# LazyLatte/vortex-raytracing

Measured on AMD Instinct MI355X. Metric: Mrays/s (primary+shadow) at 1920x1080, 1M-tri BVH, higher is better.
Workload: dtype f32; 1 GPU; configs[2]: Sponza-class 1048576 tris, 1920x1080, primary + 1 shadow ray per hit; frames_in_flight=2, frames_per_launch_group=5, parallelism=1 GPU: whole frames, 5 per set of launches (vxrt_render_batch), 2 sets in flight, world_size=1, bvh_nodes=726810, bvh_depth=13

## Files before the change

### vortex-raytracing_amd/build.py

```python
import os
import shutil
import struct
import subprocess
import sys

HERE = os.path.dirname(os.path.abspath(__file__))
CSRC = os.path.join(HERE, "csrc")
LIB = os.path.join(HERE, "lib")
VXBIN = os.path.join(HERE, "vxbin")
ROCM = os.environ.get("ROCM_PATH", "/opt/rocm")
HIPCC = os.path.join(ROCM, "bin", "hipcc")
ARCH = "gfx950"

HIP_FLAGS = ["--offload-arch=" + ARCH, "-O3", "-ffp-contract=off", "-fno-slp-vectorize", "-fPIC", "-std=c++17", "-Wall", "-Wno-unused-function"]
HIP_FLAGS += os.environ.get("VXRT_EXTRA_HIPFLAGS", "").split()
CXX_FLAGS = ["-O2", "-ffp-contract=off", "-fPIC", "-std=c++17", "-Wall"]

PRODUCT_HIP_SOURCES = ("rt_kernels.hip", "rt_accel.hip", "rt_secondary.hip", "rt_path.hip", "rt_denoise.hip", "rc_kernels.hip", "vx_backend.hip", "bvh_builder.hip")


def hip_library_deps():
    incs = sorted(f for f in os.listdir(CSRC) if f.endswith((".h", ".inc")))
    return [os.path.join(CSRC, f) for f in PRODUCT_HIP_SOURCES + tuple(incs)] + [os.path.join(HERE, "..", "include", "vortex_hip.h")]

SELECTORS = {
    "kernel": (0x80000000, "raytracing.kernel"),
    "miss": (0x80100000, "raytracing.miss"),
    "closest": (0x80200000, "raytracing.closest"),
    "anyhit": (0x80300000, "raytracing.anyhit"),
    "raycast/kernel": (0x80000000, "raycast.kernel"),
}


def _newer(target, sources):
    if not os.path.exists(target):
        return True
    t = os.path.getmtime(target)
    return any(os.path.getmtime(s) > t for s in sources)


def _run(cmd):
    print("+", " ".join(cmd), flush=True)
    subprocess.check_call(cmd)


def write_selectors():
    os.makedirs(VXBIN, exist_ok=True)
    for name, (vma, tag) in SELECTORS.items():
        payload = ("VXHIP1:" + tag).encode() + b"\0"
        payload += b"\0" * (64 - len(payload))
        blob = struct.pack("<QQ", vma, vma + 0x1000) + payload
        os.makedirs(os.path.dirname(os.path.join(VXBIN, name)), exist_ok=True)
        with open(os.path.join(VXBIN, name + ".vxbin"), "wb") as f:
            f.write(blob)


TEST_VARIANT_FLAGS = ["-DRT_TOP_NODES=84", "-DRT_LDS_STACK_RENDER=5", "-DRT_LDS_STACK_RENDER_PACKED=4", "-DRT_TRI_LDS=4", "-DRT_TRI_LDS_MIN=2", "-DRT_ORDER_CHECK=1"]


def build_test_variant(force=False):
    d = os.path.join(HERE, "lib_ab", "lds_staging")
    os.makedirs(d, exist_ok=True)
    so = os.path.join(d, "libvortex-hip.so")
    src = [os.path.join(CSRC, f) for f in PRODUCT_HIP_SOURCES]
    if force or _newer(so, hip_library_deps()):
        _run([HIPCC] + HIP_FLAGS + TEST_VARIANT_FLAGS + ["-shared", "-o", so] + src)
    for f in ("libvortex.so", "libvxrt_scene.so"):
        shutil.copy2(os.path.join(LIB, f), os.path.join(d, f))
    return d


def build(force=False, verbose=True):
    os.makedirs(LIB, exist_ok=True)
    hdrs = hip_library_deps()
    if not os.path.exists(HIPCC):
        raise RuntimeError("hipcc not found at %s: the HIP path cannot be built" % HIPCC)

    hip_so = os.path.join(LIB, "libvortex-hip.so")
    hip_src = [os.path.join(CSRC, f) for f in PRODUCT_HIP_SOURCES]
    if force or _newer(hip_so, hdrs):
        _run([HIPCC] + HIP_FLAGS + ["-shared", "-o", hip_so] + hip_src)

    cal_so = os.path.join(LIB, "libvxrt_calib.so")
    cal_src = [os.path.join(CSRC, "calib_kernels.hip")]
    if force or _newer(cal_so, cal_src):
        _run([HIPCC] + HIP_FLAGS + ["-shared", "-o", cal_so] + cal_src)

    stub_so = os.path.join(LIB, "libvortex.so")
    stub_src = [os.path.join(CSRC, "vx_stub.cpp")]
    if force or _newer(stub_so, stub_src + hdrs):
        _run(["g++"] + CXX_FLAGS + ["-shared", "-o", stub_so] + stub_src + ["-ldl"])

    scene_so = os.path.join(LIB, "libvxrt_scene.so")
    scene_src = [os.path.join(CSRC, "scene_builder.cpp")]
    if force or _newer(scene_so, scene_src + hdrs):
        _run(["g++"] + CXX_FLAGS + ["-pthread", "-shared", "-o", scene_so] + scene_src + ["-lz"])

    host = os.path.join(LIB, "rt_host")
    host_src = [os.path.join(CSRC, "rt_host.cpp")]
    if os.path.exists(host_src[0]) and (force or _newer(host, host_src + hdrs + [stub_so, scene_so])):
        _run(["g++"] + CXX_FLAGS + ["-o", host] + host_src + ["-L" + LIB, "-lvortex", "-lvxrt_scene", "-pthread", "-Wl,-rpath,$ORIGIN"])

    write_selectors()
    build_test_variant(force)
    return {"hip": hip_so, "stub": stub_so, "scene": scene_so}


if __name__ == "__main__":
    build(force="--force" in sys.argv)
```

### vortex-raytracing_amd/csrc/rt_kernels.hip

```cpp
#include <hip/hip_runtime.h>
#include <stdint.h>
#include "rt_internal.h"
#include "pinhole.h"
#include "rt_shading.h"
#include "rt_order.h"

template <bool EXACT>
__device__ __forceinline__ float slab_interval(float tx1, float tx2, float ty1, float ty2, float tz1, float tz2) {
  float tmin, tmax;
  if (EXACT) {
    tmin = std_min(tx1, tx2);
    tmax = std_max(tx1, tx2);
    tmin = std_max(tmin, std_min(ty1, ty2));
    tmax = std_min(tmax, std_max(ty1, ty2));
    tmin = std_max(tmin, std_min(tz1, tz2));
    tmax = std_min(tmax, std_max(tz1, tz2));
  } else {
    tmin = fmaxf(fmaxf(fminf(tx1, tx2), fminf(ty1, ty2)), fminf(tz1, tz2));
    tmax = fminf(fminf(fmaxf(tx1, tx2), fmaxf(ty1, ty2)), fmaxf(tz1, tz2));
  }
  return (tmax < tmin || tmax <= 0) ? RT_LARGE_FLOAT : tmin;
}

template <bool EXACT>
// ... 117 lines not shown
  }
  const uint32_t desc[4] = {q2.z, q2.w, q3.x, q3.y};
  float d[4];
  bool in[4] = {true, true, true, true};
  if constexpr (NO_SELECT) {
    static_assert(!EXACT && !LDEXP, "the select-free box test is the fast form's");
    d[0] = child_box_raw<0>(pl, px, py, pz, sx, sy, sz, rox, roy, roz, rix, riy, riz, in[0]);
    d[1] = child_box_raw<1>(pl, px, py, pz, sx, sy, sz, rox, roy, roz, rix, riy, riz, in[1]);
    d[2] = child_box_raw<2>(pl, px, py, pz, sx, sy, sz, rox, roy, roz, rix, riy, riz, in[2]);
    d[3] = child_box_raw<3>(pl, px, py, pz, sx, sy, sz, rox, roy, roz, rix, riy, riz, in[3]);
  } else {
    d[0] = child_box<0, EXACT, LDEXP>(pl, px, py, pz, sx, sy, sz, ex, ey, ez, rox, roy, roz, rix, riy, riz);
    d[1] = child_box<1, EXACT, LDEXP>(pl, px, py, pz, sx, sy, sz, ex, ey, ez, rox, roy, roz, rix, riy, riz);
    d[2] = child_box<2, EXACT, LDEXP>(pl, px, py, pz, sx, sy, sz, ex, ey, ez, rox, roy, roz, rix, riy, riz);
    d[3] = child_box<3, EXACT, LDEXP>(pl, px, py, pz, sx, sy, sz, ex, ey, ez, rox, roy, roz, rix, riy, riz);
  }
#pragma unroll
  for (int k = 0; k < 4; ++k) {
    if constexpr (NO_SELECT) ok[k] = (desc[k] != DESC_NONE) && in[k] && (d[k] < hit_dist);
    else ok[k] = (desc[k] != DESC_NONE) && (d[k] < hit_dist);
    c[k].d = d[k];
    c[k].desc = desc[k];
  }
}

template <bool EXACT, bool LDEXP>
__device__ __forceinline__ void eval_children(const uint4 q0, const uint4 q1, const uint4 q2, const uint4 q3, const uint32_t* __restrict__ ref_node,
                                              float rox, float roy, float roz, float rix, float riy, float riz,
                                              float hit_dist, Cand* c) {
  bool ok[4];
  eval_children_raw<EXACT, LDEXP>(q0, q1, q2, q3, ref_node, rox, roy, roz, rix, riy, riz, hit_dist, c, ok);
#pragma unroll
  for (int k = 0; k < 4; ++k) c[k].d = ok[k] ? c[k].d : __builtin_inff();
}

struct Fetches { unsigned node = 0, inst = 0, tri = 0; };

#define ITER_LIMIT (1u << 22)

template <int N>
__device__ __forceinline__ float* cam_lds() { __shared__ float s[N]; return s; }

#ifndef RT_TRI_PREFETCH
#define RT_TRI_PREFETCH 1
#endif
#ifndef RT_WAVES_PER_EU
#define RT_WAVES_PER_EU 6
#endif

#ifndef RT_DEAD_MAX
#define RT_DEAD_MAX 64
#endif
#ifndef RT_LEAF_MIN
#define RT_LEAF_MIN 1
#endif
#ifndef RT_TRACE_LEAF_MIN
#define RT_TRACE_LEAF_MIN 24
#endif
#ifndef RT_TRI_LDS
#define RT_TRI_LDS 0
#endif
#ifndef RT_TRI_LDS_MIN
#define RT_TRI_LDS_MIN 8
#endif
#ifndef RT_UNORDERED_OCCLUSION
#define RT_UNORDERED_OCCLUSION 1
#endif
#ifndef RT_SHADOW_FINISH_MIN
#define RT_SHADOW_FINISH_MIN 65
#endif
#ifndef RT_TRACE_DEAD_MAX
#define RT_TRACE_DEAD_MAX 16
#endif
#ifndef RT_CHUNK
#define RT_CHUNK 64
#endif
#ifndef RT_TRACE_NT
#define RT_TRACE_NT 0
#endif
#ifndef RT_TRACE_CHUNK
#define RT_TRACE_CHUNK 64
#endif
#ifndef RT_XCC_HOME
#define RT_XCC_HOME 1
#endif
#ifndef RT_QUEUE_DRY_MASK
#define RT_QUEUE_DRY_MASK 1
#endif
#ifndef RT_STEAL_SPREAD
#define RT_STEAL_SPREAD 0
#endif
#ifndef RT_WAVES_TRACE
#define RT_WAVES_TRACE 7
#endif
#ifndef RT_LDS_STACK_TRACE
#define RT_LDS_STACK_TRACE 7
#endif
#ifndef RT_WAVES_RENDER
#define RT_WAVES_RENDER 7
#endif
#ifndef RT_LDS_STACK_RENDER
#define RT_LDS_STACK_RENDER 6
#endif
#ifndef RT_WAVES_RENDER_PACKED
#define RT_WAVES_RENDER_PACKED 8
#endif
#ifndef RT_LDS_STACK_RENDER_PACKED
#define RT_LDS_STACK_RENDER_PACKED 5
#endif
#ifndef LDS_STACK
#define LDS_STACK 8
#endif
#ifndef RT_WG_WAVES
#define RT_WG_WAVES 4
#endif
#define RT_WG_THREADS (64 * RT_WG_WAVES)

enum { JOB_RENDER = 0, JOB_RENDER_SHADOW = 1, JOB_TRACE = 2, JOB_RENDER_GI = 3, JOB_TRACE_UNORDERED = 4 };
__host__ __device__ constexpr bool is_trace_job(int job) { return job == JOB_TRACE || job == JOB_TRACE_UNORDERED; }
enum { JOB_CAM = 8 };
__host__ __device__ constexpr int job_base(int job) { return job & ~JOB_CAM; }
__host__ __device__ constexpr bool is_cam_job(int job) { return (job & JOB_CAM) != 0; }
#ifndef RT_WAVES_GI
#define RT_WAVES_GI 7
#endif
#ifndef RT_LDS_STACK_GI
#define RT_LDS_STACK_GI 6
#endif
#ifndef RT_GI_DEAD_MAX
#define RT_GI_DEAD_MAX 64
#endif

#ifndef RT_BATCH_PUSH
#define RT_BATCH_PUSH 1
#endif
#ifndef RT_LEAF_FLAT
#define RT_LEAF_FLAT 1
#endif
#ifndef RT_OCC_OK_MASKS
#define RT_OCC_OK_MASKS 1
#endif
#ifndef RT_OCC_LOOP
#define RT_OCC_LOOP 1
#endif
#ifndef RT_OCC_LOOP_CHECK
#define RT_OCC_LOOP_CHECK 0
#endif
#ifndef RT_ORDER_PATHS
#define RT_ORDER_PATHS 1
#endif
#ifndef RT_ORDER_CHECK
#define RT_ORDER_CHECK 0
#endif

#ifdef RT_ISA_MARKS
#define RT_MARK(name) asm volatile("; RTMARK " name)
#else
#define RT_MARK(name)
#endif
#define RT_LOOP_MARK(name) do { if constexpr (OCC) { RT_MARK("occ_" name); } else { RT_MARK(name); } } while (0)

__device__ __forceinline__ uint32_t frame_row(uint32_t lr, uint32_t y0, uint32_t row_step) { return y0 + (lr >> 3) * row_step + (lr & 7u); }

struct FastDiv { uint32_t d, m, s; };
static FastDiv fast_div_make(uint32_t d) {
  FastDiv f{d ? d : 1u, 1u, 0u};
  while ((1ull << f.s) < f.d) ++f.s;
  f.m = (uint32_t)((((1ull << f.s) - f.d) << 32) / f.d) + 1u;
  return f;
}
__device__ __forceinline__ uint32_t fast_div(uint32_t x, const FastDiv& f) { return (__umulhi(x, f.m) + x) >> f.s; }

struct PersistArgs {
  uint32_t W, H, y0, y1, tiles_x;
  FastDiv div_tiles_x, div_frame_tiles;
  uint32_t row_step;
  uint32_t total;
  const uint32_t* total_dev;
  HitRec* hits;
  const float* rays; const float* tmax; int any_hit;
  const uint32_t* order;
  unsigned long long* counters;
  uint32_t* status;
  uint32_t* queue;
  uint32_t per_shard;
  const float* utab; const float* vtab;
  uint32_t* defer_count; uint32_t* defer_list; uint32_t defer_cap;
  const uint32_t* tile_order; uint32_t* tile_cost;
  uint32_t shard_rot;
  unsigned long long* wave_log;
  unsigned long long* end_log;
  const ShadeParams* pbatch; uint32_t frame_tiles;
  uint32_t* dst; float* colors; uint32_t gi_seed;
  const uint8_t* alpha_tri;
};

#define RT_FAST_INV_MAX 0x1p+64f
#define RT_FAST_POS_MAX 0x1p+60f
__device__ __forceinline__ bool ray_in_fast_domain(float ox, float oy, float oz, float ix, float iy, float iz) {
  return fabsf(ix) <= RT_FAST_INV_MAX && fabsf(iy) <= RT_FAST_INV_MAX && fabsf(iz) <= RT_FAST_INV_MAX && ix != 0.0f && iy != 0.0f && iz != 0.0f &&
         fabsf(ox) <= RT_FAST_POS_MAX && fabsf(oy) <= RT_FAST_POS_MAX && fabsf(oz) <= RT_FAST_POS_MAX;
}


#define F_FOUND 1u
#define F_ANYHIT 2u
#define F_SHADOW 8u
#define F_WORLD 16u
#define F_RESUMED 32u

__device__ unsigned long long g_child_counts[8];

template <int JOB, int STATS, bool LDEXP, bool EXACT, bool PACKED = false, bool SHALLOW = false, bool ALPHA = false, bool IDENT = false>
__global__ __launch_bounds__(EXACT ? 256 : RT_WG_THREADS, EXACT ? 4 : (is_trace_job(JOB) ? RT_WAVES_TRACE : (job_base(JOB) == JOB_RENDER_GI ? RT_WAVES_GI : (PACKED ? RT_WAVES_RENDER_PACKED : RT_WAVES_RENDER)))) void rt_persistent_kernel(SceneDev sc, ShadeParams p, PersistArgs A) {
  static_assert(!ALPHA || (STATS == 0 && !PACKED && !SHALLOW && job_base(JOB) != JOB_RENDER_GI), "alpha instantiations: see ALPHA above");
  static_assert(!IDENT || (STATS == 0 && !ALPHA && !EXACT && !LDEXP && SHALLOW && (job_base(JOB) == JOB_RENDER || job_base(JOB) == JOB_RENDER_SHADOW)), "identity-root instantiations: see IDENT above");
  constexpr int LSTK = EXACT ? LDS_STACK : (is_trace_job(JOB) ? RT_LDS_STACK_TRACE : (job_base(JOB) == JOB_RENDER_GI ? RT_LDS_STACK_GI : (PACKED ? RT_LDS_STACK_RENDER_PACKED : RT_LDS_STACK_RENDER)));
  constexpr int WG_WAVES = EXACT ? 4 : RT_WG_WAVES;
  constexpr bool USE_TOP = RT_TOP_NODES > 0 && !EXACT && !LDEXP;
  constexpr uint32_t DEAD_MAX = is_trace_job(JOB) ? RT_TRACE_DEAD_MAX : (job_base(JOB) == JOB_RENDER_GI ? RT_GI_DEAD_MAX : RT_DEAD_MAX);
  constexpr uint32_t FINISH_MIN = job_base(JOB) == JOB_RENDER_SHADOW ? RT_SHADOW_FINISH_MIN : 65u;
  const uint32_t lane = threadIdx.x & 63u;
  const uint32_t n_jobs = EXACT ? min(*A.defer_count, A.defer_cap) : (A.total_dev ? min(*A.total_dev, A.total) : A.total);
  const uint32_t per_shard = (EXACT || A.total_dev) ? (((n_jobs + QUEUE_SHARDS - 1) / QUEUE_SHARDS + 63u) & ~63u) : A.per_shard;

  __shared__ uint2 s_stk[WG_WAVES][LSTK][64];
  constexpr int NCTX = (!EXACT && is_trace_job(JOB)) ? 8 : 9;
  __shared__ uint32_t s_ctx[WG_WAVES][NCTX][64];
  __shared__ uint32_t s_dry;
  if (threadIdx.x == 0) s_dry = 0u;
  float* s_cam = nullptr;
  if constexpr (is_cam_job(JOB)) {
    s_cam = cam_lds<CAM_TAB>();
    for (uint32_t i = threadIdx.x; i < (uint32_t)CAM_TAB; i += blockDim.x) s_cam[i] = A.utab[i];
  }
  __syncthreads();
  uint2* const lstk = &s_stk[threadIdx.x >> 6][0][lane];
  auto lstk4_here = [&]() -> uint32_t* {
    uint32_t l = lane;
    asm volatile("" : "+v"(l));
    return (uint32_t*)lstk - l;
  };
  uint32_t* const ctx = &s_ctx[threadIdx.x >> 6][0][lane];
#define CTX(i) ctx[((NCTX == 8 && (i) > 5) ? (i) - 1 : (i)) * 64]
  __shared__ uint4 s_top[USE_TOP ? 4 : 1][USE_TOP ? RT_TOP_NODES : 1];
  constexpr bool TRI_LDS = RT_TRI_LDS > 0 && !EXACT && !is_trace_job(JOB);
  __shared__ float4 s_tri[TRI_LDS ? WG_WAVES : 1][TRI_LDS ? 3 * RT_TRI_LDS : 1];
  const uint32_t n_top = USE_TOP ? min(sc.n_top, (uint32_t)RT_TOP_NODES) : 0u;
  if (USE_TOP && n_top) {
    for (uint32_t i = threadIdx.x; i < 4u * n_top; i += (uint32_t)(64 * WG_WAVES)) s_top[i / n_top][i % n_top] = sc.top_img[(size_t)(i / n_top) * RT_TOP_NODES + (i % n_top)];
    __syncthreads();
  }
  const uint32_t root_desc = (USE_TOP && n_top) ? sc.tlas_root_top : sc.tlas_root;
  const uint32_t* const blas_roots = (USE_TOP && n_top) ? sc.blas_root_top : sc.blas_root;
  const uint32_t root_blas_desc = is_inst_desc(root_desc) ? blas_roots[root_desc & PAYLOAD_MASK] : DESC_DONE;

  float arx = 0, ary = 0, arz = 0, aix = 0, aiy = 0, aiz = 0;
  float hitd = 0, path_m = 0, tos_m = 0;
  uint32_t cur = DESC_IDLE, tos_d = DESC_DONE, job = 0, flags = 0;
  float g_col[3] = {0.f, 0.f, 0.f}, g_alb[3] = {0.f, 0.f, 0.f}, g_ray[6] = {0.f, 0.f, 0.f, 0.f, 0.f, 0.f};
  int sp = 0;
  constexpr int STACK_CAP = SHALLOW ? 3 * RT_SHALLOW_LEVELS : LSTK + RT_STACK_ENTRIES;
  static_assert(STACK_CAP > LSTK, "stack");
  uint32_t ovf_d[STACK_CAP - LSTK];
  float ovf_m[STACK_CAP - LSTK];
  constexpr bool BOX_NO_SELECT = RT_BOX_NO_SELECT && RT_OCC_OK_MASKS && IDENT && job_base(JOB) == JOB_RENDER_SHADOW;
  constexpr bool OCC_LOOP = RT_OCC_LOOP && IDENT && RT_BATCH_PUSH && RT_UNORDERED_OCCLUSION && RT_OCC_OK_MASKS && job_base(JOB) == JOB_RENDER_SHADOW &&
                            DEAD_MAX >= 64u && FINISH_MIN > 64u && STACK_CAP > 2 * LSTK;
  bool queue_empty = false;
  const uint32_t xcc_id = RT_XCC_HOME ? (uint32_t)__builtin_amdgcn_s_getreg((3 << 11) | (0 << 6) | 20) : blockIdx.x;
  const uint32_t shard = (xcc_id + A.shard_rot) % QUEUE_SHARDS;
  uint32_t tries = 0, loc_next = 0, loc_end = 0;
  uint32_t loc_off = 0;
  uint32_t lpt_tile = 0xFFFFFFFFu, lpt_work = 0; unsigned long long lpt_t0 = 0;
  Fetches fx;
  unsigned nrays = 0, nhit = 0;
  unsigned long long t_first = 0;
  unsigned long long wl_tn = 0, wl_tl = 0, wl_t0 = 0;
  unsigned wl_no23 = 0, wl_no3 = 0, wl_iter = 0, wl_node_x = 0, wl_node_l = 0, wl_leaf_x = 0, wl_leaf_l = 0;
  unsigned wl_cc[8] = {0, 0, 0, 0, 0, 0, 0, 0};
  unsigned long long wl_tstart = 0, wl_tf = 0, wl_tfin = 0, wl_tmark = 0;
  unsigned long long wl_tq = 0;
  if (STATS && A.wave_log) { t_first = wall_clock64(); wl_tstart = __builtin_readcyclecounter(); }

  auto pixel_of = [&](uint32_t r, uint32_t& x, uint32_t& y) {
    asm volatile("" : "+v"(r));
    uint32_t tile = r >> 6;
    const uint32_t l = r & 63u;
    if (A.pbatch) tile -= fast_div(tile, A.div_frame_tiles) * A.frame_tiles;
    const uint32_t ty = fast_div(tile, A.div_tiles_x);
    x = (tile - ty * A.tiles_x) * 8u + (l & 7u);
    y = A.y0 + ty * A.row_step + (l >> 3);
  };
  auto hit_slot = [&]() -> HitRec* {
    uint32_t j = job;
    asm volatile("" : "+v"(j));
    return A.hits + j;
  };
  auto pixel_ray = [&](uint32_t x, uint32_t y, float& ox, float& oy, float& oz, float& dx, float& dy, float& dz) {
    if constexpr (is_cam_job(JOB)) {
      const uint32_t f = A.pbatch ? fast_div(job >> 6, A.div_frame_tiles) : 0u;
      camera_ray(s_cam + f * CAM_HDR, A.vtab + (size_t)f * (A.W + A.H), A.W, x, y, ox, oy, oz, dx, dy, dz);
    } else generate_ray(A.utab[x], A.vtab[y], ox, oy, oz, dx, dy, dz);
  };
  auto world_ray = [&](float& ox, float& oy, float& oz, float& dx, float& dy, float& dz, float& tmax_) {
    tmax_ = RT_LARGE_FLOAT;
    if (is_trace_job(JOB)) {
      const float* rp = A.rays + (size_t)job * 6;
      if (RT_TRACE_NT) {
        ox = __builtin_nontemporal_load(rp); oy = __builtin_nontemporal_load(rp + 1); oz = __builtin_nontemporal_load(rp + 2);
        dx = __builtin_nontemporal_load(rp + 3); dy = __builtin_nontemporal_load(rp + 4); dz = __builtin_nontemporal_load(rp + 5);
      } else { ox = rp[0]; oy = rp[1]; oz = rp[2]; dx = rp[3]; dy = rp[4]; dz = rp[5]; }
      if (A.tmax) tmax_ = A.tmax[job];
    } else {
      uint32_t x, y;
      pixel_of(job, x, y);
      pixel_ray(x, y, ox, oy, oz, dx, dy, dz);
      if (job_base(JOB) == JOB_RENDER_GI && (flags & F_SHADOW)) {
        ox = g_ray[0]; oy = g_ray[1]; oz = g_ray[2]; dx = g_ray[3]; dy = g_ray[4]; dz = g_ray[5];
      }
      if (job_base(JOB) == JOB_RENDER_SHADOW && (flags & F_SHADOW)) {
        const float pd = __uint_as_float(CTX(5));
        float sox, soy, soz, sdx, sdy, sdz, sdist;
        float lpx = p.lpos[0], lpy = p.lpos[1], lpz = p.lpos[2];
        if (A.pbatch) { const ShadeParams* q = A.pbatch + fast_div(job >> 6, A.div_frame_tiles); lpx = q->lpos[0]; lpy = q->lpos[1]; lpz = q->lpos[2]; }
        shadow_ray(lpx, lpy, lpz, ox, oy, oz, dx, dy, dz, pd, sox, soy, soz, sdx, sdy, sdz, sdist);
        ox = sox; oy = soy; oz = soz; dx = sdx; dy = sdy; dz = sdz;
        tmax_ = sdist;
      }
    }
  };
  auto defer = [&](bool counted) {
    const uint32_t slot = atomicAdd(A.defer_count, 1u);
    if (job_base(JOB) == JOB_RENDER_GI && (flags & F_SHADOW)) nrays--;
    if (slot < A.defer_cap) A.defer_list[slot] = job | ((flags & F_SHADOW) && job_base(JOB) != JOB_RENDER_GI ? 0x80000000u : 0u);
    if (job_base(JOB) == JOB_RENDER_SHADOW && (flags & F_SHADOW)) {
      HitRec h;
      h.bx = __uint_as_float(CTX(3)); h.by = __uint_as_float(CTX(4)); h.bz = 1 - h.bx - h.by;
      h.dist = __uint_as_float(CTX(5)); h.blasIdx = CTX(6); h.triIdx = CTX(7);
      *hit_slot() = h;
    }
    if (counted) nrays--;
    cur = DESC_IDLE;
  };
  auto enter_instance = [&](uint32_t blasIdx, float ox, float oy, float oz, float dx, float dy, float dz) {
    const uint32_t* bp = sc.blas + (size_t)blasIdx * (RT_BLAS_STRIDE / 4);
    uint32_t bw[13];
#pragma unroll
    for (int i = 0; i < 13; ++i) bw[i] = bp[i];
    if (STATS) { fx.node++; fx.inst++; }
    const float m00 = __uint_as_float(bw[1]), m01 = __uint_as_float(bw[2]), m02 = __uint_as_float(bw[3]), m03 = __uint_as_float(bw[4]);
    const float m10 = __uint_as_float(bw[5]), m11 = __uint_as_float(bw[6]), m12 = __uint_as_float(bw[7]), m13 = __uint_as_float(bw[8]);
    const float m20 = __uint_as_float(bw[9]), m21 = __uint_as_float(bw[10]), m22 = __uint_as_float(bw[11]), m23 = __uint_as_float(bw[12]);
    arx = m00 * ox + m01 * oy + m02 * oz + m03;
    ary = m10 * ox + m11 * oy + m12 * oz + m13;
    arz = m20 * ox + m21 * oy + m22 * oz + m23;
    const float cdx = m00 * dx + m01 * dy + m02 * dz;
    const float cdy = m10 * dx + m11 * dy + m12 * dz;
    const float cdz = m20 * dx + m21 * dy + m22 * dz;
    aix = 1.0f / cdx; aiy = 1.0f / cdy; aiz = 1.0f / cdz;
    const bool s2 = ray_in_fast_domain(arx, ary, arz, aix, aiy, aiz);
    if (!EXACT && !s2) { defer(true); return; }
    flags &= ~F_WORLD;
    CTX(0) = __float_as_uint(cdx); CTX(1) = __float_as_uint(cdy); CTX(2) = __float_as_uint(cdz);
    CTX(8) = blasIdx;
    cur = blas_roots[blasIdx];
  };
  auto start_ray = [&](float ox, float oy, float oz, float dx, float dy, float dz, float tmax_, bool any_) {
    arx = ox; ary = oy; arz = oz;
    aix = 1.0f / dx; aiy = 1.0f / dy; aiz = 1.0f / dz;
    const bool safe = ray_in_fast_domain(ox, oy, oz, aix, aiy, aiz);
    flags = (flags & (F_SHADOW | F_RESUMED)) | F_WORLD | (any_ ? F_ANYHIT : 0u);
    if (!EXACT && !safe) {
      if (!is_trace_job(JOB) && !is_cam_job(JOB) && !(flags & F_SHADOW)) cur = DESC_IDLE; else defer(false);
      return;
    }
    hitd = tmax_ > RT_LARGE_FLOAT ? RT_LARGE_FLOAT : tmax_;
    path_m = -__builtin_inff(); sp = 0; tos_d = DESC_DONE;
    cur = root_desc;
    nrays++;
    if (is_inst_desc(root_desc)) {
      const bool no_neg_zero = __float_as_uint(ox) != 0x80000000u && __float_as_uint(oy) != 0x80000000u && __float_as_uint(oz) != 0x80000000u;
      if (sc.ident_root && safe && no_neg_zero) {
        if (STATS) { fx.node++; fx.inst++; }
        flags &= ~F_WORLD;
        CTX(0) = __float_as_uint(dx); CTX(1) = __float_as_uint(dy); CTX(2) = __float_as_uint(dz);
        CTX(8) = root_desc & PAYLOAD_MASK;
        cur = root_blas_desc;
      } else enter_instance(root_desc & PAYLOAD_MASK, ox, oy, oz, dx, dy, dz);
    }
  };
  volatile uint32_t* const vovf_d = ovf_d;
  volatile float* const vovf_m = ovf_m;
  auto push = [&](uint32_t d, float m) {
    if (tos_d != DESC_DONE) {
      if (sp < LSTK) lstk[sp * 64] = make_uint2(tos_d, __float_as_uint(tos_m));
      else { ovf_d[sp - LSTK] = tos_d; ovf_m[sp - LSTK] = tos_m; }
      ++sp;
    }
    tos_d = d; tos_m = m;
  };
  auto push_pending = [&](auto occ, bool p0, uint32_t d0, float m0, bool p1, uint32_t d1, float m1, bool p2, uint32_t d2, float m2) {
    constexpr bool OCC = decltype(occ)::value;
    if (!RT_BATCH_PUSH) {
      if (p0) push(d0, m0);
      if (p1) push(d1, m1);
      if (p2) push(d2, m2);
      return;
    }
    if (!(p0 || p1 || p2)) return;
    const bool w_top = tos_d != DESC_DONE;
    const bool w0 = p0 && (p1 || p2), w1 = p1 && p2;
    const int q0 = sp + (w_top ? 1 : 0), q1 = q0 + (w0 ? 1 : 0), end = q1 + (w1 ? 1 : 0);
    if constexpr (OCC) {
      constexpr int LROWS = 2 * LSTK;
      uint32_t* const lstk4 = lstk4_here();
      if (end <= LROWS) {
        if (w_top) lstk4[sp * 64] = tos_d;
        if (w0) lstk4[q0 * 64] = d0;
        if (w1) lstk4[q1 * 64] = d1;
      } else if (sp >= LROWS) {
        if (w_top) ovf_d[sp - LROWS] = tos_d;
        if (w0) ovf_d[q0 - LROWS] = d0;
        if (w1) ovf_d[q1 - LROWS] = d1;
      } else {
        auto put = [&](int q, uint32_t d) {
          if (q < LROWS) lstk4[q * 64] = d;
          else ovf_d[q - LROWS] = d;
        };
        if (w_top) put(sp, tos_d);
        if (w0) put(q0, d0);
        if (w1) put(q1, d1);
      }
    } else
    if (end <= LSTK) {
      if (w_top) lstk[sp * 64] = make_uint2(tos_d, __float_as_uint(tos_m));
      if (w0) lstk[q0 * 64] = make_uint2(d0, __float_as_uint(m0));
      if (w1) lstk[q1 * 64] = make_uint2(d1, __float_as_uint(m1));
    } else if (sp >= LSTK) {
      if (w_top) { ovf_d[sp - LSTK] = tos_d; ovf_m[sp - LSTK] = tos_m; }
      if (w0) { ovf_d[q0 - LSTK] = d0; ovf_m[q0 - LSTK] = m0; }
      if (w1) { ovf_d[q1 - LSTK] = d1; ovf_m[q1 - LSTK] = m1; }
    } else {
      auto put = [&](int q, uint32_t d, float m) {
        if (q < LSTK) lstk[q * 64] = make_uint2(d, __float_as_uint(m));
        else { ovf_d[q - LSTK] = d; ovf_m[q - LSTK] = m; }
      };
      if (w_top) put(sp, tos_d, tos_m);
      if (w0) put(q0, d0, m0);
      if (w1) put(q1, d1, m1);
    }
    sp = end;
    tos_d = p2 ? d2 : (p1 ? d1 : d0);
    if constexpr (!OCC) tos_m = p2 ? m2 : (p1 ? m1 : m0);
  };
  auto stack_load = [&](auto occ, int i, uint32_t& d, float& m) {
    if constexpr (decltype(occ)::value) {
      typedef __attribute__((address_space(3))) const uint32_t lds_u32_t;
      if (i < 2 * LSTK) d = ((lds_u32_t*)lstk4_here())[i * 64];
      else d = ovf_d[i - 2 * LSTK];
    } else {
      typedef uint32_t u32x2_t __attribute__((ext_vector_type(2)));
      typedef __attribute__((address_space(3))) const u32x2_t lds_u32x2_t;
      if (i < LSTK) { const u32x2_t e = ((lds_u32x2_t*)lstk)[i * 64]; d = e.x; m = __uint_as_float(e.y); }
      else { d = ovf_d[i - LSTK]; m = ovf_m[i - LSTK]; }
    }
  };
  auto pop_next = [&](auto occ) {
    if constexpr (decltype(occ)::value) {
      cur = tos_d;
      tos_d = DESC_DONE;
      if (cur != DESC_DONE && sp > 0) { --sp; float m; stack_load(occ, sp, tos_d, m); }
      return;
    }
    if (RT_BATCH_PUSH) {
      uint32_t d = tos_d; float m = tos_m;
      while (d != DESC_DONE && !(m < hitd)) {
        if (sp > 0) { --sp; stack_load(occ, sp, d, m); } else d = DESC_DONE;
      }
      cur = d;
      tos_d = DESC_DONE;
      if (d != DESC_DONE) {
        path_m = m;
        if (sp > 0) { --sp; stack_load(occ, sp, tos_d, tos_m); }
      }
      return;
    }
    cur = DESC_DONE;
    while (tos_d != DESC_DONE) {
      const uint32_t d = tos_d;
      const float m = tos_m;
      if (sp > 0) {
        --sp;
        if (sp < LSTK) { const uint2 e = lstk[sp * 64]; tos_d = e.x; tos_m = __uint_as_float(e.y); }
        else { tos_d = ovf_d[sp - LSTK]; tos_m = ovf_m[sp - LSTK]; }
      } else {
        tos_d = DESC_DONE;
      }
      if (m < hitd) { cur = d; path_m = m; break; }
    }
  };

  for (;;) {
    RT_MARK("fetch");
    if (STATS && A.wave_log) wl_tmark = __builtin_readcyclecounter();
    {
      const unsigned long long idle = __ballot(cur == DESC_IDLE);
      if (!queue_empty && idle != 0ull && (is_trace_job(JOB) || FINISH_MIN > 64u || idle == ~0ull || RT_DEAD_MAX < 64)) {
        const uint32_t wl_tries0 = tries; const unsigned long long wl_tpoll0 = (STATS && A.wave_log) ? __builtin_readcyclecounter() : 0ull;
        if (loc_next == loc_end) {
          uint32_t dry = RT_QUEUE_DRY_MASK ? *(volatile uint32_t*)&s_dry : 0u;
          while (tries < QUEUE_SHARDS) {
            const uint32_t step = RT_STEAL_SPREAD ? (((tries & 1u) << 2) | (tries & 2u) | ((tries >> 2) & 1u)) : tries;
            const uint32_t sid = (shard + step) % QUEUE_SHARDS;
            if (RT_QUEUE_DRY_MASK && ((dry >> sid) & 1u)) { ++tries; continue; }
            const uint32_t s_lo = sid * per_shard;
            uint32_t in_range;
            asm volatile("s_cmp_lt_u32 %1, %2\n\ts_cselect_b32 %0, 1, 0 ; RTGUARD shard_range" : "=s"(in_range)
                         : "s"(__builtin_amdgcn_readfirstlane(s_lo)), "s"(__builtin_amdgcn_readfirstlane(n_jobs)) : "scc");
            if (!in_range) { ++tries; continue; }
            const uint32_t s_n = min(per_shard, n_jobs - s_lo);
            uint32_t base = 0;
            constexpr uint32_t CHUNK = (is_trace_job(JOB) && !EXACT) ? (uint32_t)RT_TRACE_CHUNK : (uint32_t)RT_CHUNK;
            if (lane == 0) base = atomicAdd(A.queue + sid * QUEUE_STRIDE, CHUNK);
            base = __shfl(base, 0);
            if (base < s_n) {
              loc_next = s_lo + base; loc_end = s_lo + min(base + CHUNK, s_n);
              break;
            }
            if (RT_QUEUE_DRY_MASK) {
              if (lane == 0) atomicOr(&s_dry, 1u << sid);
              dry |= 1u << sid;
            }
            ++tries;
          }
          if (tries >= QUEUE_SHARDS) { queue_empty = true; if (STATS && A.wave_log && !wl_tq) wl_tq = wall_clock64(); }
          if (STATS && A.wave_log && !USE_TOP && tries != wl_tries0 && lane == 0) wl_no23 += (unsigned)(__builtin_readcyclecounter() - wl_tpoll0);
        }
        uint32_t avail = loc_end - loc_next;
        if (!is_trace_job(JOB) && !EXACT) {
          avail = min(avail, 64u - (loc_next & 63u));
          if (avail != 0u && (A.tile_order || A.tile_cost)) {
            const uint32_t pos = loc_next >> 6;
            const uint32_t tile = A.tile_order ? A.tile_order[pos] : pos;
            loc_off = __builtin_amdgcn_readfirstlane((tile << 6) - (loc_next & ~63u));
            if (A.tile_cost && tile != lpt_tile) {
              if (lane == 0 && lpt_tile != 0xFFFFFFFFu) A.tile_cost[lpt_tile] = lpt_work;
              if (STATS && A.wave_log) {
                const unsigned long long now = wall_clock64();
                if (lane == 0) {
                  if (lpt_tile != 0xFFFFFFFFu) A.tile_cost[2u * (A.total >> 6) + lpt_tile] = (uint32_t)min(now - lpt_t0, 0xFFFFFFFFull);
                  A.tile_cost[(A.total >> 6) + tile] = (uint32_t)now;
                  A.tile_cost[3u * (A.total >> 6) + tile] = tries;
                }
                lpt_t0 = now;
              }
              lpt_tile = tile; lpt_work = 0;
            }
          }
        }
        if (avail != 0u && cur == DESC_IDLE) {
          const uint32_t rank = (uint32_t)__popcll(idle & ((1ull << lane) - 1ull));
          if (rank < avail) {
            job = loc_next + rank + loc_off;
            flags = 0;
            if (!EXACT && is_trace_job(JOB) && A.order) job = A.order[job];
            if (EXACT) {
              const uint32_t wd = A.defer_list[job];
              job = wd & 0x7fffffffu;
              if (wd >> 31) { flags = F_SHADOW | F_RESUMED; if (job_base(JOB) == JOB_RENDER_SHADOW) CTX(5) = __float_as_uint(hit_slot()->dist); }
            }
            float ox, oy, oz, dx, dy, dz, tm;
            if (is_trace_job(JOB)) {
              world_ray(ox, oy, oz, dx, dy, dz, tm);
              start_ray(ox, oy, oz, dx, dy, dz, tm, A.any_hit != 0);
            } else {
              uint32_t x, y;
              pixel_of(job, x, y);
              if (x < A.W && y < A.y1) {
                world_ray(ox, oy, oz, dx, dy, dz, tm);
                start_ray(ox, oy, oz, dx, dy, dz, tm, (flags & F_SHADOW) != 0u);
              }
            }
          }
        }
        loc_next += min(avail, (uint32_t)__popcll(idle));
      }
      if (__ballot(cur != DESC_IDLE) == 0ull) {
        if (queue_empty && loc_next == loc_end) {
          if (!is_trace_job(JOB) && !EXACT && A.tile_cost && lane == 0 && lpt_tile != 0xFFFFFFFFu) {
            A.tile_cost[lpt_tile] = lpt_work;
            if (STATS && A.wave_log) A.tile_cost[2u * (A.total >> 6) + lpt_tile] = (uint32_t)min(wall_clock64() - lpt_t0, 0xFFFFFFFFull);
          }
          break;
        }
        if (STATS && A.wave_log) wl_tf += __builtin_readcyclecounter() - wl_tmark;
        continue;
      }
    }
    if (STATS && A.wave_log) wl_tf += __builtin_readcyclecounter() - wl_tmark;

    if constexpr (OCC_LOOP) {
      auto traverse = [&](auto occ) {
        constexpr bool OCC = decltype(occ)::value;
#include "rt_traverse_loop.inc"
      };
      if (RT_OCC_LOOP_CHECK && is_work_desc(cur) && (sp != 0 || tos_d != DESC_DONE)) atomicOr(A.status, STATUS_ITER_LIMIT);
      if (__all(!is_work_desc(cur) || (flags & F_ANYHIT) != 0u)) traverse(std::true_type());
      else traverse(std::false_type());
    } else {
      constexpr bool OCC = false;
      const std::false_type occ;
#include "rt_traverse_loop.inc"
    }

    RT_MARK("finish");
    if (STATS && A.wave_log) wl_tmark = __builtin_readcyclecounter();
    if (cur == DESC_DONE) {
      const bool found = (flags & F_FOUND) != 0u;
      HitRec h; h.dist = RT_LARGE_FLOAT; h.bx = 0; h.by = 0; h.bz = 0; h.blasIdx = 0; h.triIdx = 0;
      if (is_trace_job(JOB)) {
        if (found) {
          h.dist = hitd; h.bx = __uint_as_float(CTX(3)); h.by = __uint_as_float(CTX(4)); h.bz = 1 - h.bx - h.by;
          h.blasIdx = CTX(6); h.triIdx = CTX(7);
        }
        if (RT_TRACE_NT) {
          uint32_t* hp = (uint32_t*)hit_slot();
          __builtin_nontemporal_store(__float_as_uint(h.dist), hp); __builtin_nontemporal_store(__float_as_uint(h.bx), hp + 1);
          __builtin_nontemporal_store(__float_as_uint(h.by), hp + 2); __builtin_nontemporal_store(__float_as_uint(h.bz), hp + 3);
          __builtin_nontemporal_store(h.blasIdx, hp + 4); __builtin_nontemporal_store(h.triIdx, hp + 5);
        } else *hit_slot() = h;
        cur = DESC_IDLE;
      } else if (job_base(JOB) == JOB_RENDER_GI) {
        uint32_t x, y;
        pixel_of(job, x, y);
        const size_t e = (size_t)x + (size_t)y * A.W;
        bool write = false;
        float cr = 0.f, cg = 0.f, cb = 0.f;
        if (found) {
          h.dist = hitd; h.bx = __uint_as_float(CTX(3)); h.by = __uint_as_float(CTX(4)); h.bz = 1 - h.bx - h.by;
          h.blasIdx = CTX(6); h.triIdx = CTX(7);
        }
        if (!(flags & F_SHADOW)) {
          float ox, oy, oz, dx, dy, dz;
          pixel_ray(x, y, ox, oy, oz, dx, dy, dz);
          if (!found) {
            cr = p.bg[0]; cg = p.bg[1]; cb = p.bg[2];
            write = true;
          } else {
            float r, g, b, refl, Ix, Iy, Iz, Nx, Ny, Nz, a3[3];
            shade_terms<false>(sc, p, ox, oy, oz, dx, dy, dz, h, false, r, g, b, refl, Ix, Iy, Iz, Nx, Ny, Nz, nullptr, a3);
            float thr = 1.0f;
            thr *= refl;
            g_col[0] = r + p.bg[0] * thr; g_col[1] = g + p.bg[1] * thr; g_col[2] = b + p.bg[2] * thr;
            g_alb[0] = a3[0]; g_alb[1] = a3[1]; g_alb[2] = a3[2];
            ao_sample_ray(x, y, A.W, 1u, 0u, A.gi_seed, Ix, Iy, Iz, Nx, Ny, Nz, dx, dy, dz, g_ray);
            flags = F_SHADOW;
            start_ray(g_ray[0], g_ray[1], g_ray[2], g_ray[3], g_ray[4], g_ray[5], RT_LARGE_FLOAT, false);
          }
        } else {
          float r, g, b;
          shade_eval<false>(sc, p, g_ray[0], g_ray[1], g_ray[2], g_ray[3], g_ray[4], g_ray[5], h, found, false, r, g, b);
          cr = g_col[0] + g_alb[0] * r; cg = g_col[1] + g_alb[1] * g; cb = g_col[2] + g_alb[2] * b;
          write = true;
        }
        if (write) {
          A.dst[e] = pack_rgb8(cr, cg, cb);
          if (A.colors) { A.colors[3 * e] = cr; A.colors[3 * e + 1] = cg; A.colors[3 * e + 2] = cb; }
          cur = DESC_IDLE;
        }
      } else if (!(flags & F_SHADOW)) {
        if (STATS && found) nhit++;
        if (job_base(JOB) == JOB_RENDER_SHADOW && found) {
          uint32_t x, y;
          pixel_of(job, x, y);
          float ox, oy, oz, dx, dy, dz, sox, soy, soz, sdx, sdy, sdz, sdist;
          pixel_ray(x, y, ox, oy, oz, dx, dy, dz);
          float lpx = p.lpos[0], lpy = p.lpos[1], lpz = p.lpos[2];
          if (A.pbatch) { const ShadeParams* q = A.pbatch + fast_div(job >> 6, A.div_frame_tiles); lpx = q->lpos[0]; lpy = q->lpos[1]; lpz = q->lpos[2]; }
          shadow_ray(lpx, lpy, lpz, ox, oy, oz, dx, dy, dz, hitd, sox, soy, soz, sdx, sdy, sdz, sdist);
          CTX(5) = __float_as_uint(hitd);
          flags = F_SHADOW;
          start_ray(sox, soy, soz, sdx, sdy, sdz, sdist, true);
        } else {
          if (found) {
            h.dist = hitd; h.bx = __uint_as_float(CTX(3)); h.by = __uint_as_float(CTX(4)); h.bz = 1 - h.bx - h.by;
            h.blasIdx = CTX(6); h.triIdx = CTX(7);
          }
          *hit_slot() = h;
          cur = DESC_IDLE;
        }
      } else if (EXACT && (flags & F_RESUMED)) {
        if (found) hit_slot()->blasIdx |= 0x80000000u;
        cur = DESC_IDLE;
      } else {
        h.bx = __uint_as_float(CTX(3)); h.by = __uint_as_float(CTX(4)); h.bz = 1 - h.bx - h.by;
        h.dist = __uint_as_float(CTX(5)); h.blasIdx = CTX(6) | (found ? 0x80000000u : 0u); h.triIdx = CTX(7);
        *hit_slot() = h;
        cur = DESC_IDLE;
      }
    }
    if (STATS && A.wave_log) wl_tfin += __builtin_readcyclecounter() - wl_tmark;
  }
#undef CTX

  if (STATS && A.wave_log && !EXACT) {
    unsigned s = nrays;
    for (int o = 32; o > 0; o >>= 1) s += __shfl_down(s, o);
    for (int o = 32; o > 0; o >>= 1) wl_no23 += __shfl_down(wl_no23, o);
    if (lane == 0) {
      unsigned long long* w = A.wave_log + 16ull * (blockIdx.x * (uint32_t)WG_WAVES + (threadIdx.x >> 6));
      w[13] = wl_tf; w[14] = wl_tfin; w[15] = wl_tq;
      w[0] = t_first; w[1] = wall_clock64(); w[2] = s; w[8] = wl_no23;
      w[9] = (unsigned long long)wl_no3 | ((unsigned long long)(uint32_t)__builtin_amdgcn_s_getreg((3 << 11) | (0 << 6) | 20) << 56);
      w[10] = wl_tn; w[11] = wl_tl; w[12] = __builtin_readcyclecounter() - wl_tstart;
      w[3] = wl_iter; w[4] = wl_node_x; w[5] = wl_node_l; w[6] = wl_leaf_x; w[7] = wl_leaf_l;
#pragma unroll
      for (int k = 0; k < 8; ++k) if (wl_cc[k]) atomicAdd(&g_child_counts[k], (unsigned long long)wl_cc[k]);
    }
  }
  if (!EXACT && A.end_log) {
    unsigned s = nrays;
    for (int o = 32; o > 0; o >>= 1) s += __shfl_down(s, o);
    if (lane == 0) {
      unsigned long long* w = A.end_log + 2ull * (blockIdx.x * (uint32_t)WG_WAVES + (threadIdx.x >> 6));
      w[0] = wall_clock64();
      w[1] = (unsigned long long)s | ((unsigned long long)(uint32_t)__builtin_amdgcn_s_getreg((3 << 11) | (0 << 6) | 20) << 56);
    }
  }
  if (A.counters) {
    __shared__ unsigned s_cnt[5];
    if (threadIdx.x < 5u) s_cnt[threadIdx.x] = 0u;
    __syncthreads();
    unsigned v[5] = {nrays, fx.node, fx.inst, fx.tri, nhit};
#pragma unroll
    for (int k = 0; k < (STATS ? 5 : 1); ++k) {
      unsigned s = v[k];
      for (int o = 32; o > 0; o >>= 1) s += __shfl_down(s, o);
      if (lane == 0 && s) atomicAdd(&s_cnt[k], s);
    }
    __syncthreads();
    if (threadIdx.x < (STATS ? 5u : 1u) && s_cnt[threadIdx.x]) atomicAdd(A.counters + threadIdx.x, (unsigned long long)s_cnt[threadIdx.x]);
  }
}

__device__ __forceinline__ uint32_t lpt_cls(uint32_t c) {
  if (c < 64u) return c;
  const uint32_t e = 31u - (uint32_t)__clz((int)c);
  return ((e - 5u) << 6) | ((c >> (e - 6u)) & 63u);
}
__device__ void lpt_order_block(uint32_t shard, const uint32_t* __restrict__ cost, uint32_t* __restrict__ order,
                                uint32_t n_tiles, uint32_t tiles_per_shard, uint32_t* hist ,
                                const uint32_t* __restrict__ base_order = nullptr) {
  const uint32_t lo = shard * tiles_per_shard;
  const uint32_t hi = min(lo + tiles_per_shard, n_tiles);
  if (lo >= hi) return;
  const uint32_t lane = threadIdx.x & 63u, wave = threadIdx.x >> 6;
  for (uint32_t i = threadIdx.x; i < 2048u; i += 256u) hist[i] = 0u;
  __syncthreads();
  for (uint32_t t = lo + threadIdx.x; t < hi; t += 256u) atomicAdd(&hist[2047u - lpt_cls(cost[base_order ? base_order[t] : t])], 1u);
  __syncthreads();
  uint32_t v[8], sum = 0;
#pragma unroll
  for (int k = 0; k < 8; ++k) { v[k] = hist[threadIdx.x * 8u + k]; sum += v[k]; }
  uint32_t inc = sum;
  for (int o = 1; o < 64; o <<= 1) { const uint32_t y = __shfl_up(inc, o); if (lane >= (uint32_t)o) inc += y; }
  if (lane == 63u) hist[2048u + wave] = inc;
  __syncthreads();
  uint32_t base = inc - sum;
  for (uint32_t w = 0; w < wave; ++w) base += hist[2048u + w];
#pragma unroll
  for (int k = 0; k < 8; ++k) { hist[threadIdx.x * 8u + k] = base; base += v[k]; }
  __syncthreads();
  for (uint32_t t = lo + threadIdx.x; t < hi; t += 256u) {
    const uint32_t tile = base_order ? base_order[t] : t;
    order[lo + atomicAdd(&hist[2047u - lpt_cls(cost[tile])], 1u)] = tile;
  }
}

template <bool STATS, bool CAM>
__device__ __forceinline__ void shade_pass(SceneDev sc, ShadeParams p, uint32_t W, uint32_t H, uint32_t y0, uint32_t y1, uint32_t row_step,
                                           uint32_t n_rows, const float* __restrict__ utab, const float* __restrict__ vtab,
                                           const HitRec* __restrict__ hb, uint32_t* __restrict__ dst,
                                           HitRec* __restrict__ hits, float* __restrict__ colors,
                                           unsigned long long* counters, uint32_t* __restrict__ ctl_reset,
                                           uint32_t lpt_blocks, const uint32_t* __restrict__ lpt_cost, uint32_t* __restrict__ lpt_order,
                                           uint32_t lpt_tiles, uint32_t lpt_per_shard,
                                           uint32_t batch, const ShadeParams* __restrict__ pbatch, uint64_t dst_frame_stride,
                                           const uint32_t* __restrict__ lpt_base) {
  __shared__ uint32_t s_hist[2048 + 8];
  if (blockIdx.x < lpt_blocks) { lpt_order_block(blockIdx.x, lpt_cost, lpt_order, lpt_tiles, lpt_per_shard, s_hist, lpt_base); return; }
  const uint32_t blk = blockIdx.x - lpt_blocks;
  if (ctl_reset && blk == 0)
    for (uint32_t i = threadIdx.x; i < CTL_DWORDS; i += 256u) ctl_reset[i] = 0u;
  const uint64_t t = (uint64_t)blk * 256u + threadIdx.x;
  const uint64_t n = (uint64_t)W * n_rows * batch;
  unsigned ntex = 0, npix = 0;
  const uint32_t x = (uint32_t)(t % W), vr = (uint32_t)(t / W);
  const uint32_t frame = batch > 1 ? vr / n_rows : 0u, lr = vr - frame * n_rows, y = frame_row(lr, y0, row_step);
  if (batch > 1 && t < n) { p = pbatch[frame]; dst += (size_t)frame * dst_frame_stride; }
  if (t < n && y < y1) {
    const size_t idx = (size_t)x + (size_t)y * W;
    HitRec h = hb[hit_index(x, vr, (W + 7u) >> 3)];
    const uint32_t occ_bit = h.blasIdx & 0x80000000u;
    const bool occ = occ_bit != 0u;
    h.blasIdx &= 0x7fffffffu;
    const bool found = h.dist != RT_LARGE_FLOAT;
    float ox, oy, oz, dx, dy, dz;
    frame_pixel_ray<CAM>(utab, vtab, W, H, frame, x, y, ox, oy, oz, dx, dy, dz);
    float r, g, b;
    shade_eval<STATS>(sc, p, ox, oy, oz, dx, dy, dz, h, found, occ, r, g, b, &ntex);
    dst[idx] = pack_rgb8(r, g, b);
    if (hits) { HitRec o = h; o.blasIdx |= occ_bit; hits[idx] = o; }
    if (colors) { colors[3 * idx] = r; colors[3 * idx + 1] = g; colors[3 * idx + 2] = b; }
    npix = 1;
  }
  if (STATS && counters) {
    const uint32_t lane = threadIdx.x & 63u;
    unsigned v[2] = {ntex, npix};
#pragma unroll
    for (int k = 0; k < 2; ++k) {
      unsigned s = v[k];
      for (int o = 32; o > 0; o >>= 1) s += __shfl_down(s, o);
      if (lane == 0 && s) atomicAdd(counters + 5 + k, (unsigned long long)s);
    }
  }
}
template <bool STATS>
__global__ __launch_bounds__(256) void rt_shade_kernel(SceneDev sc, ShadeParams p, uint32_t W, uint32_t H, uint32_t y0, uint32_t y1, uint32_t row_step,
                                                      uint32_t n_rows, const float* __restrict__ utab, const float* __restrict__ vtab,
                                                      const HitRec* __restrict__ hb, uint32_t* __restrict__ dst,
                                                      HitRec* __restrict__ hits, float* __restrict__ colors,
// ... 1231 lines not shown
```

Baseline: 12310 Mrays/s.

## Treat render tiles as wave-uniform and reuse primary ray for shadow setup

Adds a RT_TILE_SECTIONS mode, on by default, in which the tile index is made wave-uniform with readfirstlane, so per-frame divisions and light-position loads go to scalar registers and the constant address space. Primary rays are generated directly from the pixel instead of through world_ray. Shadow-ray setup reuses the stored primary origin and direction (marked with a new F_DIRECT flag) instead of regenerating the camera ray. The lane id for the packed LDS stack comes from mbcnt. A static_assert limits the mode to the ident/shadow render configuration, and a build variant with the mode disabled is added for comparison. The risk is wrong results if a wave ever holds jobs from more than one tile.

```diff
diff --git a/vortex-raytracing_amd/build.py b/vortex-raytracing_amd/build.py
--- a/vortex-raytracing_amd/build.py
+++ b/vortex-raytracing_amd/build.py
@@ -58,13 +58,16 @@
 TEST_VARIANT_FLAGS = ["-DRT_TOP_NODES=84", "-DRT_LDS_STACK_RENDER=5", "-DRT_LDS_STACK_RENDER_PACKED=4", "-DRT_TRI_LDS=4", "-DRT_TRI_LDS_MIN=2", "-DRT_ORDER_CHECK=1"]
 
 
-def build_test_variant(force=False):
-    d = os.path.join(HERE, "lib_ab", "lds_staging")
+TILE_SECTIONS_OFF_FLAGS = ["-DRT_TILE_SECTIONS=0"]
+
+
+def build_test_variant(force=False, name="lds_staging", flags=None):
+    d = os.path.join(HERE, "lib_ab", name)
     os.makedirs(d, exist_ok=True)
     so = os.path.join(d, "libvortex-hip.so")
     src = [os.path.join(CSRC, f) for f in PRODUCT_HIP_SOURCES]
     if force or _newer(so, hip_library_deps()):
-        _run([HIPCC] + HIP_FLAGS + TEST_VARIANT_FLAGS + ["-shared", "-o", so] + src)
+        _run([HIPCC] + HIP_FLAGS + (TEST_VARIANT_FLAGS if flags is None else flags) + ["-shared", "-o", so] + src)
     for f in ("libvortex.so", "libvxrt_scene.so"):
         shutil.copy2(os.path.join(LIB, f), os.path.join(d, f))
     return d
@@ -103,6 +106,7 @@
 
     write_selectors()
     build_test_variant(force)
+    build_test_variant(force, "tile_sections_off", TILE_SECTIONS_OFF_FLAGS)
     return {"hip": hip_so, "stub": stub_so, "scene": scene_so}
 
 
diff --git a/vortex-raytracing_amd/csrc/rt_kernels.hip b/vortex-raytracing_amd/csrc/rt_kernels.hip
--- a/vortex-raytracing_amd/csrc/rt_kernels.hip
+++ b/vortex-raytracing_amd/csrc/rt_kernels.hip
@@ -293,6 +293,9 @@
 #ifndef RT_ORDER_CHECK
 #define RT_ORDER_CHECK 0
 #endif
+#ifndef RT_TILE_SECTIONS
+#define RT_TILE_SECTIONS 1
+#endif
 
 #ifdef RT_ISA_MARKS
 #define RT_MARK(name) asm volatile("; RTMARK " name)
@@ -349,6 +352,7 @@
 #define F_SHADOW 8u
 #define F_WORLD 16u
 #define F_RESUMED 32u
+#define F_DIRECT 64u
 
 __device__ unsigned long long g_child_counts[8];
 
@@ -379,6 +383,9 @@
   uint2* const lstk = &s_stk[threadIdx.x >> 6][0][lane];
   auto lstk4_here = [&]() -> uint32_t* {
     uint32_t l = lane;
+    if constexpr (RT_TILE_SECTIONS != 0 && PACKED && IDENT) {
+      asm volatile("v_mbcnt_lo_u32_b32 %0, -1, 0\n\tv_mbcnt_hi_u32_b32 %0, -1, %0" : "=v"(l));
+    } else
     asm volatile("" : "+v"(l));
     return (uint32_t*)lstk - l;
   };
@@ -424,9 +431,15 @@
   unsigned long long wl_tq = 0;
   if (STATS && A.wave_log) { t_first = wall_clock64(); wl_tstart = __builtin_readcyclecounter(); }
 
+  constexpr bool TILE_SECTIONS = RT_TILE_SECTIONS != 0 && OCC_LOOP;
+  static_assert(!TILE_SECTIONS || (IDENT && !EXACT && DEAD_MAX >= 64u && FINISH_MIN > 64u && job_base(JOB) == JOB_RENDER_SHADOW), "wave-uniform tile: see TILE_SECTIONS");
+  auto tile_of = [&](uint32_t r) -> uint32_t {
+    if constexpr (TILE_SECTIONS) return (uint32_t)__builtin_amdgcn_readfirstlane(r >> 6);
+    else return r >> 6;
+  };
   auto pixel_of = [&](uint32_t r, uint32_t& x, uint32_t& y) {
     asm volatile("" : "+v"(r));
-    uint32_t tile = r >> 6;
+    uint32_t tile = tile_of(r);
     const uint32_t l = r & 63u;
     if (A.pbatch) tile -= fast_div(tile, A.div_frame_tiles) * A.frame_tiles;
     const uint32_t ty = fast_div(tile, A.div_tiles_x);
@@ -440,7 +453,7 @@
   };
   auto pixel_ray = [&](uint32_t x, uint32_t y, float& ox, float& oy, float& oz, float& dx, float& dy, float& dz) {
     if constexpr (is_cam_job(JOB)) {
-      const uint32_t f = A.pbatch ? fast_div(job >> 6, A.div_frame_tiles) : 0u;
+      const uint32_t f = A.pbatch ? fast_div(tile_of(job), A.div_frame_tiles) : 0u;
       camera_ray(s_cam + f * CAM_HDR, A.vtab + (size_t)f * (A.W + A.H), A.W, x, y, ox, oy, oz, dx, dy, dz);
     } else generate_ray(A.utab[x], A.vtab[y], ox, oy, oz, dx, dy, dz);
   };
@@ -525,6 +538,7 @@
       if (sc.ident_root && safe && no_neg_zero) {
         if (STATS) { fx.node++; fx.inst++; }
         flags &= ~F_WORLD;
+        if constexpr (TILE_SECTIONS) flags |= F_DIRECT;
         CTX(0) = __float_as_uint(dx); CTX(1) = __float_as_uint(dy); CTX(2) = __float_as_uint(dz);
         CTX(8) = root_desc & PAYLOAD_MASK;
         cur = root_blas_desc;
@@ -719,7 +733,8 @@
               uint32_t x, y;
               pixel_of(job, x, y);
               if (x < A.W && y < A.y1) {
-                world_ray(ox, oy, oz, dx, dy, dz, tm);
+                if constexpr (TILE_SECTIONS) { pixel_ray(x, y, ox, oy, oz, dx, dy, dz); tm = RT_LARGE_FLOAT; }
+                else world_ray(ox, oy, oz, dx, dy, dz, tm);
                 start_ray(ox, oy, oz, dx, dy, dz, tm, (flags & F_SHADOW) != 0u);
               }
             }
@@ -813,12 +828,24 @@
       } else if (!(flags & F_SHADOW)) {
         if (STATS && found) nhit++;
         if (job_base(JOB) == JOB_RENDER_SHADOW && found) {
-          uint32_t x, y;
-          pixel_of(job, x, y);
           float ox, oy, oz, dx, dy, dz, sox, soy, soz, sdx, sdy, sdz, sdist;
-          pixel_ray(x, y, ox, oy, oz, dx, dy, dz);
+          if (TILE_SECTIONS && (flags & F_DIRECT)) {
+            ox = arx; oy = ary; oz = arz;
+            dx = __uint_as_float(CTX(0)); dy = __uint_as_float(CTX(1)); dz = __uint_as_float(CTX(2));
+          } else {
+            uint32_t x, y;
+            pixel_of(job, x, y);
+            pixel_ray(x, y, ox, oy, oz, dx, dy, dz);
+          }
           float lpx = p.lpos[0], lpy = p.lpos[1], lpz = p.lpos[2];
-          if (A.pbatch) { const ShadeParams* q = A.pbatch + fast_div(job >> 6, A.div_frame_tiles); lpx = q->lpos[0]; lpy = q->lpos[1]; lpz = q->lpos[2]; }
+          if (A.pbatch) {
+            const ShadeParams* q = A.pbatch + fast_div(tile_of(job), A.div_frame_tiles);
+            if constexpr (TILE_SECTIONS) {
+              typedef __attribute__((address_space(4))) const float cfloat_t;
+              cfloat_t* lp = (cfloat_t*)(uintptr_t)q->lpos;
+              lpx = lp[0]; lpy = lp[1]; lpz = lp[2];
+            } else { lpx = q->lpos[0]; lpy = q->lpos[1]; lpz = q->lpos[2]; }
+          }
           shadow_ray(lpx, lpy, lpz, ox, oy, oz, dx, dy, dz, hitd, sox, soy, soz, sdx, sdy, sdz, sdist);
           CTX(5) = __float_as_uint(hitd);
           flags = F_SHADOW;
```

Result: no change. 12420 Mrays/s (median of 6 runs) (+0.9%).
